# Anaesthesiaye/sound_event_detection_transformer

Measured on AMD Instinct MI355X. Metric: audio clips/sec training throughput (B=64, 10s@64-mel), higher is better.
Workload: dtype bf16; 1 GPU; URBAN-SED SEDT enc_layers=3 dec_at num_queries=10 B=64/GPU, 10 s @ 64-mel (B,1,500,64), full train step: fwd + Hungarian matching (device) + SetCriterion + bwd + clip 0.1 + AdamW, dropout 0.1; global_batch=64, parallelism=dp1

## Files before the change

### include/sedt_hip.h

```cpp
#ifndef SEDT_HIP_H
#define SEDT_HIP_H
#include <stddef.h>
#include <stdint.h>

#ifdef __cplusplus
extern "C" {
#endif

#define SEDT_F32 0
#define SEDT_BF16 1
#define SEDT_BF16X3 2
#define SEDT_I16 3

#define SEDT_ACT_NONE 0
#define SEDT_ACT_RELU 1
#define SEDT_ACT_SIGMOID 2

const char* sedt_last_error(void);
int sedt_version(void);

typedef struct SedtIgemm {
  int32_t M, N, K;
  const void* A;
  const void* B;
// ... 210 lines not shown
int sedt_bneck_fwd(const void* x, void* y, const void* w1_frag, const void* w2_frag, const void* w3_frag, const float* s1, const float* b1,
                   const float* s2, const float* b2, const float* s3, const float* b3, void* a_out, void* b_out, uint8_t* abits_out,
                   uint8_t* bbits_out, uint8_t* bits_out, int cin, int planes, int W, int B, int H, void* stream);
int sedt_bneck_bwd(const void* gy, void* gx, const void* w3t_frag, const void* w2t_frag, const void* w1t_frag, const uint8_t* abits,
                   const uint8_t* bbits, const uint8_t* xbits, void* gb_out, void* ga_out, int cin, int planes, int W, int B, int H,
                   void* stream);

int sedt_bneck3_ok(int cin, int planes, int W, int stride, int dil, int has_downsample, int B, int H, int dtype);
int sedt_bneck3_fwd(const void* x, void* y, const void* w1_frag, const void* w2_frag, const void* w3_frag, const float* s1, const float* b1,
                    const float* s2, const float* b2, const float* s3, const float* b3, void* a_out, void* b_out, uint8_t* abits_out,
                    uint8_t* bbits_out, uint8_t* bits_out, int B, int H, const SedtPrefetch* pf, void* stream);
int sedt_bneck3_bwd(const void* gy, void* gx, const void* w3t_frag, const void* w2t_frag, const void* w1t_frag, const uint8_t* abits,
                    const uint8_t* bbits, const uint8_t* xbits, void* gb_out, void* ga_out, int B, int H, const SedtPrefetch* pf,
                    void* stream);

int sedt_bneck0_ok(int cin, int planes, int W, int stride, int dil, int has_downsample, int dtype);
int sedt_bneck0_fwd(const void* x, void* y, const void* w1_frag, const void* w2_frag, const void* w3_frag, const void* wd_frag, const float* s1,
                    const float* b1, const float* s2, const float* b2, const float* s3, const float* b3, const float* sd, const float* bd,
                    void* a_out, void* b_out, uint8_t* abits_out, uint8_t* bbits_out, uint8_t* bits_out, int B, int H, void* stream);

int sedt_bneck2_ok(int cin, int planes, int W, int stride, int dil, int has_downsample, int dtype);
int sedt_bneck2_fwd(const void* x, void* y, const void* w1_frag, const void* w2_frag, const void* w3_frag, const void* wd_frag, const float* s1,
                    const float* b1, const float* s2, const float* b2, const float* s3, const float* b3, const float* sd, const float* bd,
                    void* a_out, void* b_out, uint8_t* bits_out, int B, int H, void* stream);

int sedt_heads_slab_ok(int D, int C1, int CA, int dtype);
int sedt_heads_fwd(const void* x, const float* wc, const float* bc, const void* w1_frag, const float* b1, const void* w2_frag,
                   const float* b2, const float* w3, const float* b3, const float* wa, const float* ba, float* cls, float* box, float* at,
                   void* h1, void* h2, int L, int B, int Qp, int C1, int CA, void* stream);
size_t sedt_heads_bwd_part_floats(int L, int B, int Qp, int C1, int CA);
int sedt_heads_bwd(const void* x, const void* h1, const void* h2, const float* box, const float* at, const float* g_cls,
                   const float* g_box, const float* g_at, const float* wc, const float* w3, const float* wa, const void* w2t_frag,
                   const void* w1t_frag, void* dhs, void* g_h1, void* g_h2, float* part, int L, int B, int Qp, int C1, int CA, void* stream);

int sedt_encoder_ffn_bwd(const void* gx2, const void* h, const void* x1, const float* mean2, const float* rstd2,
                         const float* gamma2, const void* w2t_frag, const void* w1t_frag, const void* wot_frag, void* g2, void* gh,
                         void* gx1, void* g1, void* gctx, float* ln_part, int B, int S, int FF, float drop_p, uint32_t seed_f,
                         uint32_t seed_o, const uint32_t* seed_ptr, void* stream);
int sedt_encoder_qkv_bwd(const void* dqk, const void* dv, const void* x, const float* mean1, const float* rstd1,
                         const float* gamma1, const void* gx1, const void* wint_frag, void* gx, float* ln_part, int B, int S,
                         void* stream);
int sedt_encoder_qkv_fwd(const void* x, const void* pos, const float* gamma, const float* beta, const void* w_in_frag,
                         const float* b_in, void* qk, void* v, void* xn, void* xnp, float* mean, float* rstd, int B, int S,
                         const SedtPrefetch* pf, void* stream);
int sedt_encoder_attn_ffn_fwd(const void* x, const void* qk, const void* v, const uint8_t* kpm, const void* w_o_frag,
                              const float* b_o, const float* gamma2, const float* beta2, const void* w1_frag, const float* b1,
                              const void* w2_frag, const float* b2, void* x2, void* ctx, float* lse, void* x1, float* mean2,
                              float* rstd2, void* x1n, void* h, int B, int S, int FF, float drop_p, uint32_t seed_attn,
                              uint32_t seed_o, uint32_t seed_h, uint32_t seed_f, const uint32_t* seed_ptr, void* stream);

int sedt_multi_gather(const SedtChunk* table, int nchunks, int mode, void* stream);
int sedt_multi_ema(const SedtChunk* table, int nchunks, float decay, const int32_t* guard , void* stream);
int sedt_multi_sumsq(const SedtChunk* table, int nchunks, float* partial, float* sumsq, int32_t* step_ptr ,
                     int32_t* guard , uint32_t* seed_word , void* stream);
int sedt_multi_adamw(const SedtChunk* table, int nchunks, const float* sumsq, float max_norm, float beta1, float beta2,
                     float eps, const int32_t* step_ptr , const int32_t* guard ,
                     void* stream);

#define SEDT_CRIT_MAXL 8
#define SEDT_CRIT_MAXOUT (4 * SEDT_CRIT_MAXL + 6)
#define SEDT_CRIT_MAXCARD 8192
typedef struct SedtCriterion {
  const float* logits;
  const float* boxes;
  const float* at;
  const float* tc;
// ... 189 lines not shown
```

### sound_event_detection_transformer_amd/_build.py

```python
import os
import shutil
import subprocess
from concurrent.futures import ThreadPoolExecutor

HERE = os.path.dirname(os.path.abspath(__file__))
CSRC = os.path.join(HERE, 'csrc')
LIB = os.path.join(HERE, 'libsedt_hip.so')
OBJ = os.path.join(HERE, '..', 'build', 'obj')
SOURCES = ['igemm.hip', 'igemm3.hip', 'wgrad3.hip', 'wgrad4.hip', 'misc.hip', 'stem.hip', 'conv3x3_c64.hip',
           'norm_attn.hip', 'attn_mfma.hip', 'attn_f32_mfma.hip', 'enc_slab.hip', 'heads_slab.hip', 'bneck.hip', 'bneck3.hip', 'criterion.hip', 'postproc.hip', 'input.hip', 'skinny.hip', 'split3.hip', 'pool_at.hip', 'metrics.hip', 'decode.hip', 'psds.hip', 'sweep.hip', 'stitch.hip', 'recmetrics.hip', 'recpsds.hip', 'mel.hip', 'resample.hip', 'clips.hip', 'mixplan.hip', 'host.cpp']
FLAGS = ['--offload-arch=gfx950', '-O3', '-std=c++17', '-fPIC', '-Wno-pass-failed']
if os.environ.get('SEDT_DEV_BUILD') == '1':
    FLAGS = FLAGS + ['-DSEDT_DEV']
    LIB = os.path.join(HERE, '..', 'build', 'dev', 'libsedt_hip_dev.so')
    OBJ = os.path.join(HERE, '..', 'build', 'dev', 'obj')


def source_stamp():
    import hashlib
    h = hashlib.sha256()
    files = [os.path.join(CSRC, f) for f in sorted(os.listdir(CSRC)) if f.endswith(('.hip', '.h', '.cpp'))]
    files.append(os.path.join(HERE, '..', 'include', 'sedt_hip.h'))
    for d, _, fs in sorted(os.walk(HERE)):
        if '__pycache__' in d or os.sep + 'csrc' in d:
            continue
        files += [os.path.join(d, f) for f in sorted(fs) if f.endswith('.py')]
    for f in files:
        h.update(os.path.relpath(f, HERE).encode())
        with open(f, 'rb') as fh:
            h.update(fh.read())
    return h.hexdigest()[:16]


def _headers():
    hs = [os.path.join(CSRC, f) for f in os.listdir(CSRC) if f.endswith('.h')]
    return hs + [os.path.join(HERE, '..', 'include', 'sedt_hip.h'), os.path.abspath(__file__)]


def _newer(target, deps):
    if not os.path.exists(target):
        return True
    t = os.path.getmtime(target)
    return any(os.path.getmtime(d) > t for d in deps if os.path.exists(d))
# ... 51 lines not shown
```

### sound_event_detection_transformer_amd/functional.py

```python
import torch
from torch.autograd import Function

from . import ops, packing, runtime
from .lib import F32, BF16
from .ops import ACT_NONE, ACT_RELU, ACT_SIGMOID, ConvGeom


def _dt_of(t):
    return F32 if t.dtype == torch.float32 else BF16


def _as(t, dt):
    want = torch.float32 if dt == F32 else torch.bfloat16
    t = t.contiguous()
    return t if t.dtype == want else ops.cast(t, dt)


def _wf(dt, w):
    return w if dt == F32 else ops.cast(w, BF16)


def _wb(dt, w):
    return ops.pack_conv(dt, w, want_fwd=False)[1]

# ... 415 lines not shown
    d_win = ops._sink(w_in, (3 * E, E))
    if d_win is None:
        d_win = torch.empty((3 * E, E), device=g_out.device, dtype=torch.float32)
    d_bin = torch.empty((3 * E,), device=g_out.device, dtype=torch.float32)
    wb = s['wb_in']
    g_q = g_k = g_v = None
    dgrads = []
    if s['same_qk']:
        ops.linear_wgrad(dt, dqk, s['q_in'], out=d_win[:2 * E], bias_out=d_bin[:2 * E], batch=batch)
        if need_q or need_k:
            dgrads.append(('q', dqk, wb[:, :2 * E]))
    else:
        ops.linear_wgrad(dt, dq, s['q_in'], out=d_win[:E], bias_out=d_bin[:E], batch=batch)
        ops.linear_wgrad(dt, dk, s['k_in'], out=d_win[E:2 * E], bias_out=d_bin[E:2 * E], batch=batch)
        if need_q:
            dgrads.append(('q', dq, wb[:, :E]))
        if need_k and not kv_fused:
            dgrads.append(('k', dk, wb[:, E:2 * E]))
    ops.linear_wgrad(dt, dv, s['v_in'], out=d_win[2 * E:], bias_out=d_bin[2 * E:], batch=batch)
    if kv_fused and not s['same_qk']:
        dgrads.append(('v', dkv, wb[:, E:], {} if res_kv is None else dict(res=res_kv, ldr=res_kv.stride(0))))
    elif need_v:
        dgrads.append(('v', dv, wb[:, 2 * E:]))
    if dgrads:
        got = dict(zip([d[0] for d in dgrads], ops.linear_group(dt, [(d[1], d[2], dict(d[3]) if len(d) > 3 else {}) for d in dgrads])))
        g_q, g_k, g_v = got.get('q'), got.get('k'), got.get('v')
    return g_q, g_k, g_v, d_win, d_bin, d_wo, d_bo


def _ffn_fwd(dt, x_in, w1, b1, w2, b2, res, p, seeds, train=True, out=None, act='relu'):
    sp = runtime.seed_ptr(x_in.device) if p > 0 else None
    wf1, wb1 = _prep_linear(dt, w1, train)
    wf2, wb2 = _prep_linear(dt, w2, train)
    if act == 'gelu':
        h_pre = ops.linear(dt, x_in, wf1, bias=b1)
        h = ops.gelu_fwd(dt, h_pre, p, seeds[0], sp)
        out = ops.linear(dt, h, wf2, out, bias=b2, drop_p=p, seed=seeds[1], seed_ptr=sp, res=res, ldr=res.stride(0))
        return out, dict(x_in=x_in, h=h, h_pre=h_pre, p=p, seeds=seeds, wb1=wb1, wb2=wb2)
    h = ops.linear(dt, x_in, wf1, bias=b1, act=ACT_RELU, drop_p=p, seed=seeds[0], seed_ptr=sp)
    out = ops.linear(dt, h, wf2, out, bias=b2, drop_p=p, seed=seeds[1], seed_ptr=sp, res=res, ldr=res.stride(0))
    return out, dict(x_in=x_in, h=h, p=p, seeds=seeds, wb1=wb1, wb2=wb2)


def _ffn_bwd(dt, s, g_out, w1, w2, res_for_gx=None, batch=None, g_dropped=None):
    p = s['p']
    if g_dropped is not None:
        g2 = g_dropped
    else:
        g2 = ops.dropout_grad(dt, g_out, p, s['seeds'][1], runtime.seed_ptr(g_out.device)) if p > 0 else g_out
    d_b2 = torch.empty((g2.shape[1],), device=g2.device, dtype=torch.float32)
    d_w2 = ops.linear_wgrad(dt, g2, s['h'], bias_out=d_b2, batch=batch, param=w2)
    if s.get('h_pre') is not None:
        gh = ops.gelu_bwd(dt, ops.linear(dt, g2, s['wb2']), s['h_pre'], p, s['seeds'][0], runtime.seed_ptr(g2.device) if p > 0 else None)
    else:
        gh = ops.linear(dt, g2, s['wb2'], mask=s['h'], ldm=s['h'].stride(0), alpha=1.0 / (1.0 - p) if p > 0 else 1.0)
    d_b1 = torch.empty((gh.shape[1],), device=gh.device, dtype=torch.float32)
    d_w1 = ops.linear_wgrad(dt, gh, s['x_in'], bias_out=d_b1, batch=batch, param=w1)
    if res_for_gx is not None:
        gx = ops.linear(dt, gh, s['wb1'], res=res_for_gx, ldr=res_for_gx.stride(0))
    else:
        gx = ops.linear(dt, gh, s['wb1'])
    return gx, d_w1, d_b1, d_w2, d_b2


class EncoderLayerFn(Function):

    @staticmethod
    def forward(ctx, x, pos, kpm, amask, cfg, *P):
        dt = cfg['dt']
        (w_in, b_in, w_o, b_o, w1, b1, w2, b2, g1, be1, g2, be2) = P
        B, S, H = cfg['B'], cfg['S'], cfg['H']
        p = cfg['dropout'] if cfg['training'] else 0.0
        seeds = [runtime.next_seed() for _ in range(4)]
        x = _as(x, dt)
        pos = _as(pos, dt)
        sv = {}
        tr = any(ctx.needs_input_grad)
        fr = None
# ... 411 lines not shown
```

### sound_event_detection_transformer_amd/lib.py

```python
import ctypes as C
import os

import torch

HERE = os.path.dirname(os.path.abspath(__file__))
LIB_PATH = os.path.join(HERE, 'libsedt_hip.so')
if os.environ.get('SEDT_LIB_AB') and os.environ.get('SEDT_DEV') == '1':
    LIB_PATH = os.environ['SEDT_LIB_AB']

F32, BF16 = 0, 1
BF16X3 = 2
I16 = 3
RESAMPLE_BLK = 1024
RESAMPLE_DESC_WORDS = 6
CLIPS_MAXB = 1024
GEMM_X3 = False


def gemm_dtype(dtype):
    return BF16X3 if (dtype == F32 and GEMM_X3) else dtype
ACT_NONE, ACT_RELU, ACT_SIGMOID = 0, 1, 2
TORCH_DTYPE = {F32: torch.float32, BF16: torch.bfloat16}


# ... 115 lines not shown
    'sedt_spsedt_dec_in': (_i, [_vp, _vp, _vp, _vp, _vp, _i, _i, _i, _i, _i, _i, _f, _u32, _vp, _i, _vp]),
    'sedt_spsedt_dec_in_bwd': (_i, [_vp, _vp, _vp, _vp, _i, _i, _i, _i, _i, _i, _i, _vp]),
    'sedt_gelu_fwd': (_i, [_vp, _vp, _i64, _f, _u32, _vp, _i, _vp]),
    'sedt_gelu_bwd': (_i, [_vp, _vp, _vp, _i64, _f, _u32, _vp, _i, _vp]),
    'sedt_sigmoid_grad': (_i, [_vp, _vp, _vp, _i64, _vp]),
    'sedt_layernorm_fwd': (_i, [_vp, _vp, _vp, _vp, _vp, _vp, _vp, _vp, _i, _i, _i, _vp]),
    'sedt_layernorm_bwd': (_i, [_vp, _vp, _vp, _vp, _vp, _vp, _vp, _vp, _vp, _vp, _vp, _sz, _i, _i, _i, _vp]),
    'sedt_layernorm_bwd_scratch': (_sz, [_i, _i]),
    'sedt_layernorm_bwd_drop': (_i, [_vp, _vp, _vp, _vp, _vp, _vp, _vp, _vp, _vp, _vp, _vp, _vp, _sz, _i, _i, _vp, _f, _u32, _vp, _i, _vp]),
    'sedt_layernorm_bwd_final': (_i, [_vp, _i, _i, _vp, _vp, _vp]),
    'sedt_attention_fwd': (_i, [_vp, _i64, _vp, _i64, _vp, _i64, _vp, _i64, _vp, _vp, _vp, _i, _i, _i, _i, _f, _u32,
                                _vp, _i, _vp]),
    'sedt_attention_bwd': (_i, [_vp, _i64, _vp, _i64, _vp, _i64, _vp, _i64, _vp, _i64, _vp, _vp, _vp, _vp, _i64, _vp,
                                _i64, _vp, _i64, _i, _i, _i, _i, _f, _u32, _vp, _i, _vp]),
    'sedt_attention_describe': (_i, [_vp, _i64] * 8 + [_i, _i, _i, _f, _i, _i, C.c_char_p, _i]),
    'sedt_pack_frag': (_i, [_vp, _i, _i, _vp]),
    'sedt_encoder_slab_ok': (_i, [_i, _i, _i, _i, _i]),
    'sedt_encoder_qkv_fwd': (_i, [_vp] * 12 + [_i, _i, C.POINTER(SedtPrefetch), _vp]),
    'sedt_encoder_attn_ffn_fwd': (_i, [_vp] * 20 + [_i, _i, _i, _f, _u32, _u32, _u32, _u32, _vp, _vp]),
    'sedt_bneck_ok': (_i, [_i] * 7),
    'sedt_bneck3_ok': (_i, [_i] * 9),
    'sedt_bneck3_fwd': (_i, [_vp] * 16 + [_i, _i, C.POINTER(SedtPrefetch), _vp]),
    'sedt_bneck3_bwd': (_i, [_vp] * 10 + [_i, _i, C.POINTER(SedtPrefetch), _vp]),
    'sedt_bneck0_ok': (_i, [_i] * 7),
    'sedt_bneck2_ok': (_i, [_i] * 7),
    'sedt_bneck2_fwd': (_i, [_vp] * 17 + [_i, _i, _vp]),
    'sedt_bneck0_fwd': (_i, [_vp] * 19 + [_i, _i, _vp]),
    'sedt_bneck_fwd': (_i, [_vp] * 16 + [_i] * 5 + [_vp]),
    'sedt_bneck_bwd': (_i, [_vp] * 10 + [_i] * 5 + [_vp]),
    'sedt_heads_slab_ok': (_i, [_i, _i, _i, _i]),
    'sedt_heads_fwd': (_i, [_vp] * 16 + [_i] * 5 + [_vp]),
    'sedt_heads_bwd_part_floats': (_sz, [_i] * 5),
    'sedt_heads_bwd': (_i, [_vp] * 17 + [_i] * 5 + [_vp]),
    'sedt_encoder_ffn_bwd': (_i, [_vp] * 15 + [_i, _i, _i, _f, _u32, _u32, _vp, _vp]),
    'sedt_encoder_qkv_bwd': (_i, [_vp] * 10 + [_i, _i, _vp]),
    'sedt_posenc': (_i, [_vp, _vp, _i, _i, _i, _i, _i, _vp]),
    'sedt_mask_resize': (_i, [_vp, _vp, _i, _i, _i, _i, _i, _vp]),
    'sedt_bn_fold': (_i, [_vp, _vp, _vp, _vp, _vp, _vp, _i, _vp]),
    'sedt_pack_conv': (_i, [_vp, _i, _i, _i, _vp, _vp, _vp, _i, _vp]),
    'sedt_stem_prep': (_i, [_vp, _vp, _vp, _vp, _i, _vp]),
    'sedt_stem_im2col': (_i, [_vp, _vp, _i, _i, _i, _i, _vp]),
    'sedt_stem_conv0_grad': (_i, [_vp, _vp, _vp, _vp, _vp]),
    'sedt_conv3x3_c64': (_i, [_vp, _vp, _i, _vp, _vp, _i, _vp, _vp, _i, _i, _i, _i, _vp]),
    'sedt_stem_pool_fwd': (_i, [_vp, _vp, _vp, _vp, _vp, _vp, _vp, _i, _i, _i, _vp]),
    'sedt_stem_pool_wgrad_slabs': (_i, [_i, _i]),
    'sedt_stem_pool_wgrad': (_i, [_vp, _vp, _vp, _vp, _vp, _i, _i, _i, _i, _vp]),
    'sedt_maxpool_fwd': (_i, [_vp, _vp, _vp, _i, _i, _i, _i, _i, _vp]),
    'sedt_maxpool_bwd': (_i, [_vp, _vp, _vp, _vp, _i, _i, _i, _i, _i, _vp]),
    'sedt_maxpool_bwd_y': (_i, [_vp, _vp, _vp, _vp, _vp, _i, _i, _i, _i, _i, _vp]),
    'sedt_avgpool': (_i, [_vp, _vp, _i, _i, _i, _i, _vp]),
    'sedt_sumsq': (_i, [_vp, _i64, _vp, _vp, _sz, _i, _vp]),
    'sedt_sumsq_scratch': (_sz, [_i64]),
    'sedt_multi_bn_fold': (_i, [_vp, _i, _vp]),
    'sedt_multi_pack': (_i, [_vp, _i, _i, _i, _vp]),
    'sedt_multi_gather': (_i, [_vp, _i, _i, _vp]),
    'sedt_multi_ema': (_i, [_vp, _i, _f, _vp, _vp]),
    'sedt_multi_sumsq': (_i, [_vp, _i, _vp, _vp, _vp, _vp, _vp, _vp]),
    'sedt_multi_adamw': (_i, [_vp, _i, _vp, _f, _f, _f, _f, _vp, _vp, _vp]),
    'sedt_set_criterion_scratch': (_sz, [_i, _i, _i]),
    'sedt_set_criterion': (_i, [C.POINTER(SedtCriterion), _vp, _vp]),
    'sedt_set_criterion_bwd': (_i, [C.POINTER(SedtCriterion), _vp, _vp, _vp, _vp, _vp, _vp, _vp]),
    'sedt_match_targets': (_i, [C.POINTER(SedtMatch), _vp]),
    'sedt_feature_loss': (_i, [_vp, _vp, _vp, _vp, _vp, C.POINTER(C.c_int32), _vp, _i, _i, _i, _i, _i, _i, _vp, _vp, _vp, _vp, _vp, _vp, _vp]),
    'sedt_scale_layers': (_i, [_vp, _vp, _vp, _vp, C.POINTER(C.c_int32), _i, _i64, _vp]),
    'sedt_sum_f32': (_i, [_vp, _i, _vp, _vp]),
    'sedt_pool_at': (_i, [C.POINTER(SedtPoolAt), _vp, _vp]),
# ... 80 lines not shown
```

### sound_event_detection_transformer_amd/ops.py

```python
import ctypes as C

import os
import numpy as np
import torch

from . import lib as L
from .lib import F32, BF16, ACT_NONE, ACT_RELU, ACT_SIGMOID, TORCH_DTYPE, p as _p


class ConvGeom(object):
    __slots__ = ('Hi', 'Wi', 'Ci', 'Ho', 'Wo', 'Co', 'KH', 'KW', 'sh', 'sw', 'ph', 'pw', 'dh', 'dw')

    def __init__(self, Hi, Wi, Ci, Co, k=1, stride=1, pad=0, dil=1):
        self.Hi, self.Wi, self.Ci, self.Co = Hi, Wi, Ci, Co
        self.KH = self.KW = k
        self.sh = self.sw = stride
        self.ph = self.pw = pad
        self.dh = self.dw = dil
        self.Ho = (Hi + 2 * pad - dil * (k - 1) - 1) // stride + 1
        self.Wo = (Wi + 2 * pad - dil * (k - 1) - 1) // stride + 1

    @property
    def taps(self):
        return self.KH * self.KW
# ... 1218 lines not shown

HEADS_SLAB_MAX_ROWS = 12288


def heads_slab_ok(dtype, D, C1, CA, rows=0):
    return bool(SLAB_HEADS and dtype == BF16 and rows <= HEADS_SLAB_MAX_ROWS and L.load().sedt_heads_slab_ok(D, C1, CA, dtype))


def heads_fwd(x, wc, bc, w1f, b1, w2f, b2, w3, b3, wa, ba, Lh, B, Qp, train=True):
    _dev_check(x, wc, w3)
    rows, D = x.shape
    assert x.is_contiguous() and rows == Lh * B * Qp and wc.is_contiguous() and w3.is_contiguous() and (wa is None or wa.is_contiguous())
    C1, CA = wc.shape[0], 0 if wa is None else wa.shape[0]
    f32 = dict(device=x.device, dtype=torch.float32)
    cls, box = torch.empty((rows, C1), **f32), torch.empty((rows, 2), **f32)
    at = torch.empty((B, CA), **f32) if CA else None
    hh = (torch.empty_like(x), torch.empty_like(x)) if train else None
    L.check(L.load().sedt_heads_fwd(_p(x), _p(wc), _p(bc), _p(w1f), _p(b1), _p(w2f), _p(b2), _p(w3), _p(b3), _p(wa), _p(ba), _p(cls), _p(box),
                                    _p(at), _p(hh[0]) if hh else None, _p(hh[1]) if hh else None, Lh, B, Qp, C1, CA, L.stream_ptr()), 'heads_fwd')
    return cls, box, at, hh


def heads_bwd(x, h1, h2, box, at, g_cls, g_box, g_at, wc, w3, wa, w2t, w1t, Lh, B, Qp):
    rows, D = x.shape
    C1, CA = wc.shape[0], 0 if wa is None else wa.shape[0]
    dhs, g_h1, g_h2 = torch.empty_like(x), torch.empty_like(x), torch.empty_like(x)
    nsl = (rows + 31) // 32
    part = torch.empty((nsl, (C1 + CA + 2) * 257), device=x.device, dtype=torch.float32)
    for g in (g_cls, g_box, g_at):
        assert g is None or (g.dtype == torch.float32 and g.is_contiguous())
    L.check(L.load().sedt_heads_bwd(_p(x), _p(h1), _p(h2), _p(box), _p(at), _p(g_cls), _p(g_box), _p(g_at), _p(wc), _p(w3), _p(wa), _p(w2t),
                                    _p(w1t), _p(dhs), _p(g_h1), _p(g_h2), _p(part), Lh, B, Qp, C1, CA, L.stream_ptr()), 'heads_bwd')
    return dhs, g_h1, g_h2, part


def encoder_ffn_bwd(gx2, h, x1, mean2, rstd2, gamma2, w2t_frag, w1t_frag, wot_frag, B, S, drop_p=0.0, seeds=(0, 0), seed_ptr=None):
    _dev_check(gx2, h, x1)
    M, D = gx2.shape
    FF = h.shape[1]
    assert gx2.is_contiguous() and h.is_contiguous() and x1.is_contiguous() and M == B * S
    nsl = B * ((S + 31) // 32)
    g2 = torch.empty_like(gx2) if drop_p > 0 else None
    g1 = torch.empty_like(gx2) if drop_p > 0 else None
    gh = torch.empty_like(h)
    gx1, gctx = torch.empty_like(gx2), torch.empty_like(gx2)
    part = torch.empty((nsl, 2 * D), device=gx2.device, dtype=torch.float32)
    L.check(L.load().sedt_encoder_ffn_bwd(_p(gx2), _p(h), _p(x1), _p(mean2), _p(rstd2), _p(gamma2), _p(w2t_frag), _p(w1t_frag),
                                          _p(wot_frag), _p(g2), _p(gh), _p(gx1), _p(g1), _p(gctx), _p(part), B, S, FF, drop_p,
                                          seeds[0] & 0xffffffff, seeds[1] & 0xffffffff, _p(seed_ptr), L.stream_ptr()), 'encoder_ffn_bwd')
    return (g2 if g2 is not None else gx2), gh, gx1, (g1 if g1 is not None else gx1), gctx, part


def encoder_qkv_bwd(dqk, dv, x, mean1, rstd1, gamma1, gx1, wint_frag, B, S):
    _dev_check(dqk, dv, x, gx1)
    M, D = x.shape
    assert dqk.is_contiguous() and dv.is_contiguous() and x.is_contiguous() and gx1.is_contiguous() and M == B * S
    gx = torch.empty_like(x)
    part = torch.empty((B * ((S + 31) // 32), 2 * D), device=x.device, dtype=torch.float32)
    L.check(L.load().sedt_encoder_qkv_bwd(_p(dqk), _p(dv), _p(x), _p(mean1), _p(rstd1), _p(gamma1), _p(gx1), _p(wint_frag), _p(gx),
                                          _p(part), B, S, L.stream_ptr()), 'encoder_qkv_bwd')
    return gx, part


def posenc(dtype, mask_u8, D):
    B, H, W = mask_u8.shape
    pos = torch.empty((B, H * W, D), device=mask_u8.device, dtype=TORCH_DTYPE[dtype])
# ... 557 lines not shown
```

### sound_event_detection_transformer_amd/sedt/sedt.py

```python
import torch
from torch import nn

from .. import functional as Fn
from .. import ops, packing, runtime
from ..ops import ACT_NONE, ACT_RELU, ACT_SIGMOID
from ..utilities.utils import NestedTensor, nested_tensor_from_tensor_list


class HipLinear(nn.Linear):

    def forward(self, x, act=ACT_NONE, out_f32=False):
        lead = x.shape[:-1]
        y = Fn.LinearFn.apply(x.reshape(-1, x.shape[-1]), self.weight, self.bias, act, out_f32, runtime.compute_dtype())
        return y.view(*lead, self.out_features)


class HipConv1x1(nn.Conv2d):

    relu_input = False
    input_bits = None

    def forward(self, x):
        B, C, H, W = x.shape
        tok = x.permute(0, 2, 3, 1).reshape(B * H * W, C)
# ... 46 lines not shown
        self.dec_at = dec_at
        self.pooling = pooling
        if self.dec_at:
            self.query_embed = nn.Embedding(num_queries + 1, hidden_dim)
            self.weak_class_embed = HipLinear(hidden_dim, num_classes)
        else:
            self.query_embed = nn.Embedding(num_queries, hidden_dim)
        if self.pool_mode == 'attn':
            self.attn_dense_softmax = HipLinear(hidden_dim, num_classes)

    def pack_plan(self):
        dt, dev = runtime.compute_dtype(), self.query_embed.weight.device
        key = (dt, str(dev))
        plans = self.__dict__.setdefault('_plans', {})
        if key not in plans:
            def factory():
                body = self.backbone[0].body
                convs = []
                l34 = set(id(p_) for layer in (body.layer3, body.layer4) for p_ in layer.parameters())
                bn_only = [(body.conv1.weight, body.bn1.tensors())]
                for layer in (body.layer1, body.layer2, body.layer3, body.layer4):
                    for b in layer:
                        convs += [(b.conv1.weight, b.bn1.tensors()), (b.conv2.weight, b.bn2.tensors()), (b.conv3.weight, b.bn3.tensors())]
                        if b.downsample is not None:
                            convs.append((b.downsample[0].weight, b.downsample[1].tensors()))
                lin = [self.input_proj.weight]
                frags = []
                for l in self.transformer.encoder.layers:
                    lin += [l.self_attn.in_proj_weight, l.self_attn.out_proj.weight, l.linear1.weight, l.linear2.weight]
                    frags += [l.self_attn.in_proj_weight, l.self_attn.out_proj.weight, l.linear1.weight, l.linear2.weight]
                for l in self.transformer.decoder.layers:
                    lin += [l.self_attn.in_proj_weight, l.self_attn.out_proj.weight, l.multihead_attn.in_proj_weight,
                            l.multihead_attn.out_proj.weight, l.linear1.weight, l.linear2.weight]
                    frags += [l.self_attn.in_proj_weight, l.self_attn.out_proj.weight, l.multihead_attn.in_proj_weight,
                              l.multihead_attn.out_proj.weight, l.linear1.weight, l.linear2.weight]
                lin += [self.class_embed.weight] + [m.weight for m in self.bbox_embed.layers]
                frags += [m.weight for m in self.bbox_embed.layers[:2]]
                for name in ('weak_class_embed', 'patch2query', 'attn_dense_softmax'):
                    if hasattr(self, name):
                        lin.append(getattr(self, name).weight)
                if hasattr(self, 'feature_align'):
                    lin += [m.weight for m in self.feature_align.layers]
                cfr = [w for layer in (body.layer1, body.layer2, body.layer3) for b in layer if b.downsample is None
                       for w in (b.conv1.weight, b.conv2.weight, b.conv3.weight)]
                for b0 in (body.layer1[0], body.layer2[0]):
                    cfr += [b0.conv1.weight, b0.conv2.weight, b0.conv3.weight, b0.downsample[0].weight]
                if ops.IGEMM_BREG:
                    have = set(id(w) for w in cfr)
                    cfr += [w for w, _ in convs if id(w) not in have and id(w) in l34]
                return packing.PackPlan(dt, dev, convs, lin, bn_only, frags, cfr)
            plans[key] = packing.PlanSet(factory)
        return plans[key]

    def forward(self, samples):
        with self.pack_plan():
            return self._forward(samples)

    def _forward(self, samples):
        if isinstance(samples, (list, torch.Tensor)):
            samples = nested_tensor_from_tensor_list(samples)
        features, pos = self.backbone(samples)
        src, mask = features[-1].decompose()
        assert mask is not None
        out = {}
        hs, memory = self.transformer(self.input_proj(src), mask, self.query_embed.weight, pos[-1], enc_at_embed=None)
        q0 = 1 if self.dec_at else 0
        b = self.bbox_embed.layers
        wa = (self.weak_class_embed.weight, self.weak_class_embed.bias) if self.dec_at else (None, None)
# ... 553 lines not shown
```

Before: 13070 clips/s.

## Fuse small-M transformer FFN pair into one split-FF kernel for fwd and bwd

Adds a fused kernel that computes linear1+ReLU+dropout and linear2+dropout+residual in one launch for small row counts (decoder FFN with few queries). Work is split across four FF-quarter blocks per 32-row slab, with the last-arriving block reducing the fp32 partials. A matching backward kernel fuses the dgrad through both linears and the ReLU mask, and weight grads still use the existing wgrad path. This targets launch overhead and the h round trip for tiny decoder GEMMs. It adds counter-based cross-block reduction and partial-buffer traffic, and drops fragment packing for the decoder attention weights.

```diff
diff --git a/include/sedt_hip.h b/include/sedt_hip.h
--- a/include/sedt_hip.h
+++ b/include/sedt_hip.h
@@ -266,6 +266,15 @@
 int sedt_heads_bwd(const void* x, const void* h1, const void* h2, const float* box, const float* at, const float* g_cls,
                    const float* g_box, const float* g_at, const float* wc, const float* w3, const float* wa, const void* w2t_frag,
                    const void* w1t_frag, void* dhs, void* g_h1, void* g_h2, float* part, int L, int B, int Qp, int C1, int CA, void* stream);
+
+int sedt_ffn_pair_ok(int D, int FF, int dtype);
+size_t sedt_ffn_pair_part_floats(int M);
+int sedt_ffn_pair_fwd(const void* x, int64_t ldx, const void* res, int64_t ldr, const void* w1_frag, const float* b1, const void* w2_frag,
+                      const float* b2, void* h, void* out, int64_t ldo, float* part, uint32_t* cnt, int M, int FF, float drop_p,
+                      uint32_t seed_h, uint32_t seed_f, const uint32_t* seed_ptr, void* stream);
+int sedt_ffn_pair_bwd(const void* g, int64_t ldg, int g_is_dropped, const void* h, const void* w2t_frag, const void* w1t_frag, void* g2,
+                      void* gh, const void* res, int64_t ldr, void* gx, float* part, uint32_t* cnt, int M, int FF, float drop_p,
+                      uint32_t seed_f, const uint32_t* seed_ptr, void* stream);
 
 int sedt_encoder_ffn_bwd(const void* gx2, const void* h, const void* x1, const float* mean2, const float* rstd2,
                          const float* gamma2, const void* w2t_frag, const void* w1t_frag, const void* wot_frag, void* g2, void* gh,
diff --git a/sound_event_detection_transformer_amd/_build.py b/sound_event_detection_transformer_amd/_build.py
--- a/sound_event_detection_transformer_amd/_build.py
+++ b/sound_event_detection_transformer_amd/_build.py
@@ -8,7 +8,7 @@
 LIB = os.path.join(HERE, 'libsedt_hip.so')
 OBJ = os.path.join(HERE, '..', 'build', 'obj')
 SOURCES = ['igemm.hip', 'igemm3.hip', 'wgrad3.hip', 'wgrad4.hip', 'misc.hip', 'stem.hip', 'conv3x3_c64.hip',
-           'norm_attn.hip', 'attn_mfma.hip', 'attn_f32_mfma.hip', 'enc_slab.hip', 'heads_slab.hip', 'bneck.hip', 'bneck3.hip', 'criterion.hip', 'postproc.hip', 'input.hip', 'skinny.hip', 'split3.hip', 'pool_at.hip', 'metrics.hip', 'decode.hip', 'psds.hip', 'sweep.hip', 'stitch.hip', 'recmetrics.hip', 'recpsds.hip', 'mel.hip', 'resample.hip', 'clips.hip', 'mixplan.hip', 'host.cpp']
+           'norm_attn.hip', 'attn_mfma.hip', 'attn_f32_mfma.hip', 'enc_slab.hip', 'ffn_pair.hip', 'heads_slab.hip', 'bneck.hip', 'bneck3.hip', 'criterion.hip', 'postproc.hip', 'input.hip', 'skinny.hip', 'split3.hip', 'pool_at.hip', 'metrics.hip', 'decode.hip', 'psds.hip', 'sweep.hip', 'stitch.hip', 'recmetrics.hip', 'recpsds.hip', 'mel.hip', 'resample.hip', 'clips.hip', 'mixplan.hip', 'host.cpp']
 FLAGS = ['--offload-arch=gfx950', '-O3', '-std=c++17', '-fPIC', '-Wno-pass-failed']
 if os.environ.get('SEDT_DEV_BUILD') == '1':
     FLAGS = FLAGS + ['-DSEDT_DEV']
diff --git a/sound_event_detection_transformer_amd/csrc/ffn_pair.hip b/sound_event_detection_transformer_amd/csrc/ffn_pair.hip
--- /dev/null
+++ b/sound_event_detection_transformer_amd/csrc/ffn_pair.hip
@@ -0,0 +1,357 @@
+#include "slab.h"
+
+namespace sedt {
+
+using slab::u32x4;
+using slab::XP;
+
+constexpr int FP_D = 256;
+constexpr int FP_NQ = 4;
+constexpr int FP_NT = 512;
+constexpr int FP_SP = FP_D + 4;
+constexpr size_t FP_TILES = (size_t)2 * 32 * XP * sizeof(bf16_t);
+constexpr size_t FP_SUMT = (size_t)32 * FP_SP * sizeof(float);
+constexpr size_t FP_FLAG_OFF = FP_TILES > FP_SUMT ? FP_TILES : FP_SUMT;
+constexpr size_t FP_LDS = FP_FLAG_OFF + 16;
+
+struct FfnPairArgs {
+  const bf16_t* xin; long ldx;
+  const bf16_t* res; long ldr;
+  const u32x4* wa;
+  const u32x4* wb;
+  const float* b1; const float* b2;
+  bf16_t* h;
+  bf16_t* out; long ldo;
+  bf16_t* g2;
+  bf16_t* gh;
+  float* part;
+  unsigned* cnt;
+  int M, FF;
+  int drop_in;
+  float drop_p;
+  uint32_t thresh, seed_h, seed_f;
+  const uint32_t* seed_ptr;
+};
+
+__device__ __forceinline__ int quarter_tile(int FF, int g, int i) { return ((g >> 1) * (FF >> 7) + i) * 2 + (g & 1); }
+
+__device__ __forceinline__ void load_w_first(u32x4 (&w)[16], const u32x4* __restrict__ W, int tile, int lane) {
+  const u32x4* p = W + (long)tile * (16 * 64) + lane;
+#pragma unroll
+  for (int u = 0; u < 16; ++u) w[u] = p[u * 64];
+}
+
+__device__ __forceinline__ void load_w_second(u32x4 (&w)[16], const u32x4* __restrict__ W, int FF, int g, int i0, int nv, int wave, int lane) {
+  const u32x4* p = W + (long)wave * (FF / 16) * 64 + lane;
+#pragma unroll
+  for (int ii = 0; ii < 8; ++ii) {
+    if (ii < nv) {
+      const long ks = (long)quarter_tile(FF, g, i0 + ii) * 2;
+      w[2 * ii] = p[ks * 64];
+      w[2 * ii + 1] = p[(ks + 1) * 64];
+    }
+  }
+}
+
+__device__ __forceinline__ void gemm_first(f32x16& acc, const u32x4 (&w)[16], const bf16_t* xs, int lane) {
+  const bf16_t* xrow = xs + (lane & 31) * XP + 8 * (lane >> 5);
+#pragma unroll
+  for (int u = 0; u < 16; ++u)
+    acc = __builtin_amdgcn_mfma_f32_32x32x16_bf16(__builtin_bit_cast(bf16x8, w[u]), *reinterpret_cast<const bf16x8*>(xrow + u * 16), acc, 0, 0, 0);
+}
+
+__device__ __forceinline__ void gemm_second(f32x16& acc, const u32x4 (&w)[16], const bf16_t* hs, int nv, int lane) {
+  const bf16_t* hrow = hs + (lane & 31) * XP + 8 * (lane >> 5);
+#pragma unroll
+  for (int ii = 0; ii < 8; ++ii) {
+    if (ii < nv) {
+#pragma unroll
+      for (int q = 0; q < 2; ++q)
+        acc = __builtin_amdgcn_mfma_f32_32x32x16_bf16(__builtin_bit_cast(bf16x8, w[2 * ii + q]),
+                                                      *reinterpret_cast<const bf16x8*>(hrow + ii * 32 + q * 16), acc, 0, 0, 0);
+    }
+  }
+}
+
+__device__ __forceinline__ long part_off(int nslab, int g, int sl, int tile, int g4, int lane) {
+  return (((((long)g * nslab + sl) * 8 + tile) * 4 + g4) * 64 + lane) * 4;
+}
+
+__device__ __forceinline__ void store_partial(const f32x16& acc, float* __restrict__ part, int nslab, int g, int sl, int wave, int lane) {
+#pragma unroll
+  for (int g4 = 0; g4 < 4; ++g4)
+    slab::store_sc1(part + part_off(nslab, g, sl, wave, g4, lane),
+                    slab::f32x4_t{acc[4 * g4 + 0], acc[4 * g4 + 1], acc[4 * g4 + 2], acc[4 * g4 + 3]});
+}
+
+__device__ __forceinline__ void sum_partials(const float* __restrict__ part, int nslab, int sl, float* SUM, int wave, int lane) {
+  const int n = lane & 31, hf = lane >> 5;
+  float4 v[4];
+#pragma unroll
+  for (int g4 = 0; g4 < 4; ++g4) v[g4] = *reinterpret_cast<const float4*>(part + part_off(nslab, 0, sl, wave, g4, lane));
+#pragma unroll
+  for (int g = 1; g < FP_NQ; ++g) {
+#pragma unroll
+    for (int g4 = 0; g4 < 4; ++g4) {
+      const float4 a = *reinterpret_cast<const float4*>(part + part_off(nslab, g, sl, wave, g4, lane));
+      v[g4].x += a.x; v[g4].y += a.y; v[g4].z += a.z; v[g4].w += a.w;
+    }
+  }
+#pragma unroll
+  for (int g4 = 0; g4 < 4; ++g4) *reinterpret_cast<float4*>(SUM + n * FP_SP + wave * 32 + 8 * g4 + 4 * hf) = v[g4];
+}
+
+template <bool TRAIN>
+__global__ __launch_bounds__(FP_NT) void ffn_pair_fwd_kernel(const FfnPairArgs a) {
+  extern __shared__ __attribute__((aligned(16))) unsigned char smem[];
+  bf16_t* X = reinterpret_cast<bf16_t*>(smem);
+  bf16_t* H = X + 32 * XP;
+  float* SUM = reinterpret_cast<float*>(smem);
+  unsigned* FLAG = reinterpret_cast<unsigned*>(smem + FP_FLAG_OFF);
+  const int tid = threadIdx.x, lane = tid & 63, wave = tid >> 6, n = lane & 31, hf = lane >> 5;
+  const int nslab = (a.M + 31) / 32;
+  const int g = blockIdx.x & 3, sl = blockIdx.x >> 2;
+  const int T = a.FF >> 7;
+  const long row0 = (long)sl * 32;
+  const int nvalid = min(32, a.M - (int)row0);
+  const float inv_keep = a.thresh ? 1.f / (1.f - a.drop_p) : 1.f;
+  const uint32_t sd_off = a.seed_ptr ? *a.seed_ptr : 0u;
+  const uint32_t sd_h = a.seed_h + sd_off, sd_f = a.seed_f + sd_off;
+  uint4 xr[2];
+#pragma unroll
+  for (int q = 0; q < 2; ++q) {
+    const int u = tid + q * FP_NT, r = u >> 5, c = (u & 31) * 8;
+    xr[q] = r < nvalid ? *reinterpret_cast<const uint4*>(a.xin + (row0 + r) * a.ldx + c) : make_uint4(0, 0, 0, 0);
+  }
+  u32x4 w1[16], w2[16];
+  if (wave < T) load_w_first(w1, a.wa, quarter_tile(a.FF, g, wave), lane);
+  load_w_second(w2, a.wb, a.FF, g, 0, min(8, T), wave, lane);
+  slab::issue_fence();
+#pragma unroll
+  for (int q = 0; q < 2; ++q) {
+    const int u = tid + q * FP_NT, r = u >> 5, c = (u & 31) * 8;
+    *reinterpret_cast<uint4*>(X + r * XP + c) = xr[q];
+  }
+  __syncthreads();
+  f32x16 acc2;
+#pragma unroll
+  for (int r = 0; r < 16; ++r) acc2[r] = 0.f;
+  for (int i0 = 0; i0 < T; i0 += 8) {
+    const int nv = min(8, T - i0);
+    if (wave < nv) {
+      const int t1 = quarter_tile(a.FF, g, i0 + wave);
+      float4 bb[4];
+      slab::load_feat4(bb, a.b1, t1, hf);
+      f32x16 acc;
+#pragma unroll
+      for (int r = 0; r < 16; ++r) acc[r] = 0.f;
+      gemm_first(acc, w1, X, lane);
+      if (i0 + 8 + wave < T) load_w_first(w1, a.wa, quarter_tile(a.FF, g, i0 + 8 + wave), lane);
+#pragma unroll
+      for (int g4 = 0; g4 < 4; ++g4) {
+        const int fl = 8 * g4 + 4 * hf;
+        const float bv[4] = {bb[g4].x, bb[g4].y, bb[g4].z, bb[g4].w};
+        const uint64_t idx = (uint64_t)(row0 + n) * a.FF + t1 * 32 + fl;
+        uint32_t keep = 0xfu;
+        if (a.thresh) keep = drop_keep4(slab::inner0(sd_h), 0u, sd_h, idx, a.thresh);
+        VecT<bf16_t, 4> o;
+#pragma unroll
+        for (int e = 0; e < 4; ++e) {
+          float v = fmaxf(acc[4 * g4 + e] + bv[e], 0.f);
+          if (a.thresh) v = (keep >> e & 1u) ? v * inv_keep : 0.f;
+          o.v[e] = (bf16_t)(n < nvalid ? v : 0.f);
+        }
+        *reinterpret_cast<VecT<bf16_t, 4>*>(H + n * XP + wave * 32 + fl) = o;
+      }
+    }
+    __syncthreads();
+    if (TRAIN) {
+      for (int u = tid; u < nv * 32 * 4; u += FP_NT) {
+        const int ii = u >> 7, r = (u >> 2) & 31, c = (u & 3) * 8;
+        if (r < nvalid)
+          *reinterpret_cast<uint4*>(a.h + (row0 + r) * a.FF + quarter_tile(a.FF, g, i0 + ii) * 32 + c) =
+              *reinterpret_cast<const uint4*>(H + r * XP + ii * 32 + c);
+      }
+    }
+    gemm_second(acc2, w2, H, nv, lane);
+    if (i0 + 8 < T) load_w_second(w2, a.wb, a.FF, g, i0 + 8, min(8, T - i0 - 8), wave, lane);
+    __syncthreads();
+  }
+  store_partial(acc2, a.part, nslab, g, sl, wave, lane);
+  if (!slab::arrive_last(a.cnt + sl, FP_NQ, FLAG, tid)) return;
+  sum_partials(a.part, nslab, sl, SUM, wave, lane);
+  __syncthreads();
+  for (int u = tid; u < 1024; u += FP_NT) {
+    const int r = u >> 5, c = (u & 31) * 8;
+    if (r >= nvalid) continue;
+    const float4 s0 = *reinterpret_cast<const float4*>(SUM + r * FP_SP + c), s1 = *reinterpret_cast<const float4*>(SUM + r * FP_SP + c + 4);
+    const float4 b0 = *reinterpret_cast<const float4*>(a.b2 + c), b1v = *reinterpret_cast<const float4*>(a.b2 + c + 4);
+    float v[8] = {s0.x + b0.x, s0.y + b0.y, s0.z + b0.z, s0.w + b0.w, s1.x + b1v.x, s1.y + b1v.y, s1.z + b1v.z, s1.w + b1v.w};
+    const bf16x8 xv = *reinterpret_cast<const bf16x8*>(a.res + (row0 + r) * a.ldr + c);
+    if (a.thresh) {
+      const uint32_t keep = drop_keep8(sd_f, (uint64_t)(row0 + r) * FP_D + c, a.thresh);
+#pragma unroll
+      for (int e = 0; e < 8; ++e) v[e] = (keep >> e & 1u) ? v[e] * inv_keep : 0.f;
+    }
+    bf16x8 o;
+#pragma unroll
+    for (int e = 0; e < 8; ++e) o[e] = (bf16_t)(v[e] + (float)xv[e]);
+    *reinterpret_cast<bf16x8*>(a.out + (row0 + r) * a.ldo + c) = o;
+  }
+}
+
+__global__ __launch_bounds__(FP_NT) void ffn_pair_bwd_kernel(const FfnPairArgs a) {
+  extern __shared__ __attribute__((aligned(16))) unsigned char smem[];
+  bf16_t* G2 = reinterpret_cast<bf16_t*>(smem);
+  bf16_t* GH = G2 + 32 * XP;
+  float* SUM = reinterpret_cast<float*>(smem);
+  unsigned* FLAG = reinterpret_cast<unsigned*>(smem + FP_FLAG_OFF);
+  const int tid = threadIdx.x, lane = tid & 63, wave = tid >> 6, n = lane & 31, hf = lane >> 5;
+  const int nslab = (a.M + 31) / 32;
+  const int g = blockIdx.x & 3, sl = blockIdx.x >> 2;
+  const int T = a.FF >> 7;
+  const long row0 = (long)sl * 32;
+  const int nvalid = min(32, a.M - (int)row0);
+  const float inv_keep = a.thresh ? 1.f / (1.f - a.drop_p) : 1.f;
+  const uint32_t sd_f = a.seed_f + (a.seed_ptr ? *a.seed_ptr : 0u);
+  bf16x8 gin[2];
+#pragma unroll
+  for (int q = 0; q < 2; ++q) {
+    const int u = tid + q * FP_NT, r = u >> 5, c = (u & 31) * 8;
+#pragma unroll
+    for (int e = 0; e < 8; ++e) gin[q][e] = (bf16_t)0.f;
+    if (r < nvalid) gin[q] = *reinterpret_cast<const bf16x8*>(a.xin + (row0 + r) * a.ldx + c);
+  }
+  u32x4 w2t[16], w1t[16];
+  if (wave < T) load_w_first(w2t, a.wa, quarter_tile(a.FF, g, wave), lane);
+  load_w_second(w1t, a.wb, a.FF, g, 0, min(8, T), wave, lane);
+  slab::issue_fence();
+#pragma unroll
+  for (int q = 0; q < 2; ++q) {
+    const int u = tid + q * FP_NT, r = u >> 5, c = (u & 31) * 8;
+    bf16x8 o = gin[q];
+    if (a.drop_in && r < nvalid) {
+      const long base = (row0 + r) * FP_D + c;
+      const uint32_t keep = drop_keep8(sd_f, (uint64_t)base, a.thresh);
+#pragma unroll
+      for (int e = 0; e < 8; ++e) o[e] = (keep >> e & 1u) ? (bf16_t)((float)gin[q][e] * inv_keep) : (bf16_t)0.f;
+      if (a.g2 && g == 0) *reinterpret_cast<bf16x8*>(a.g2 + base) = o;
+    }
+    *reinterpret_cast<bf16x8*>(G2 + r * XP + c) = o;
+  }
+  __syncthreads();
+  f32x16 acc2;
+#pragma unroll
+  for (int r = 0; r < 16; ++r) acc2[r] = 0.f;
+  for (int i0 = 0; i0 < T; i0 += 8) {
+    const int nv = min(8, T - i0);
+    if (wave < nv) {
+      const int t2 = quarter_tile(a.FF, g, i0 + wave);
+      VecT<bf16_t, 4> hv[4];
+#pragma unroll
+      for (int g4 = 0; g4 < 4; ++g4) {
+        hv[g4] = VecT<bf16_t, 4>{};
+        if (n < nvalid) hv[g4] = *reinterpret_cast<const VecT<bf16_t, 4>*>(a.h + (row0 + n) * a.FF + t2 * 32 + 8 * g4 + 4 * hf);
+      }
+      f32x16 acc;
+#pragma unroll
+      for (int r = 0; r < 16; ++r) acc[r] = 0.f;
+      gemm_first(acc, w2t, G2, lane);
+      if (i0 + 8 + wave < T) load_w_first(w2t, a.wa, quarter_tile(a.FF, g, i0 + 8 + wave), lane);
+#pragma unroll
+      for (int g4 = 0; g4 < 4; ++g4) {
+        VecT<bf16_t, 4> o;
+#pragma unroll
+        for (int e = 0; e < 4; ++e) o.v[e] = (bf16_t)(((float)hv[g4].v[e] > 0.f ? acc[4 * g4 + e] : 0.f) * inv_keep);
+        *reinterpret_cast<VecT<bf16_t, 4>*>(GH + n * XP + wave * 32 + 8 * g4 + 4 * hf) = o;
+      }
+    }
+    __syncthreads();
+    for (int u = tid; u < nv * 32 * 4; u += FP_NT) {
+      const int ii = u >> 7, r = (u >> 2) & 31, c = (u & 3) * 8;
+      if (r < nvalid)
+        *reinterpret_cast<uint4*>(a.gh + (row0 + r) * a.FF + quarter_tile(a.FF, g, i0 + ii) * 32 + c) =
+            *reinterpret_cast<const uint4*>(GH + r * XP + ii * 32 + c);
+    }
+    gemm_second(acc2, w1t, GH, nv, lane);
+    if (i0 + 8 < T) load_w_second(w1t, a.wb, a.FF, g, i0 + 8, min(8, T - i0 - 8), wave, lane);
+    __syncthreads();
+  }
+  store_partial(acc2, a.part, nslab, g, sl, wave, lane);
+  if (!slab::arrive_last(a.cnt + sl, FP_NQ, FLAG, tid)) return;
+  sum_partials(a.part, nslab, sl, SUM, wave, lane);
+  __syncthreads();
+  for (int u = tid; u < 1024; u += FP_NT) {
+    const int r = u >> 5, c = (u & 31) * 8;
+    if (r >= nvalid) continue;
+    const float4 s0 = *reinterpret_cast<const float4*>(SUM + r * FP_SP + c), s1 = *reinterpret_cast<const float4*>(SUM + r * FP_SP + c + 4);
+    float v[8] = {s0.x, s0.y, s0.z, s0.w, s1.x, s1.y, s1.z, s1.w};
+    if (a.res) {
+      const bf16x8 xv = *reinterpret_cast<const bf16x8*>(a.res + (row0 + r) * a.ldr + c);
+#pragma unroll
+      for (int e = 0; e < 8; ++e) v[e] += (float)xv[e];
+    }
+    bf16x8 o;
+#pragma unroll
+    for (int e = 0; e < 8; ++e) o[e] = (bf16_t)v[e];
+    *reinterpret_cast<bf16x8*>(a.out + (row0 + r) * a.ldo + c) = o;
+  }
+}
+
+static int ffn_pair_launch(bool bwd, bool train, const FfnPairArgs& a, hipStream_t st) {
+  static_assert(FP_LDS <= 64 * 1024, "LDS");
+  const int grid = ((a.M + 31) / 32) * FP_NQ;
+  if (bwd) hipLaunchKernelGGL(ffn_pair_bwd_kernel, dim3(grid), dim3(FP_NT), FP_LDS, st, a);
+  else if (train) hipLaunchKernelGGL(ffn_pair_fwd_kernel<true>, dim3(grid), dim3(FP_NT), FP_LDS, st, a);
+  else hipLaunchKernelGGL(ffn_pair_fwd_kernel<false>, dim3(grid), dim3(FP_NT), FP_LDS, st, a);
+  return check_launch(bwd ? "ffn_pair_bwd" : "ffn_pair_fwd");
+}
+
+static bool aligned16(const void* p) { return (reinterpret_cast<uintptr_t>(p) & 15u) == 0; }
+
+}
+
+using namespace sedt;
+
+extern "C" int sedt_ffn_pair_ok(int D, int FF, int dtype) { return dtype == SEDT_BF16 && D == FP_D && FF >= 256 && FF % 256 == 0; }
+
+extern "C" size_t sedt_ffn_pair_part_floats(int M) { return (size_t)FP_NQ * ((size_t)(M + 31) / 32) * 32 * FP_D; }
+
+extern "C" int sedt_ffn_pair_fwd(const void* x, int64_t ldx, const void* res, int64_t ldr, const void* w1_frag, const float* b1,
+                                 const void* w2_frag, const float* b2, void* h, void* out, int64_t ldo, float* part, uint32_t* cnt, int M,
+                                 int FF, float drop_p, uint32_t seed_h, uint32_t seed_f, const uint32_t* seed_ptr, void* stream) {
+  SEDT_REQUIRE(x && res && w1_frag && b1 && w2_frag && b2 && out && part && cnt, "ffn_pair_fwd: null pointer");
+  SEDT_REQUIRE(M >= 1 && sedt_ffn_pair_ok(FP_D, FF, SEDT_BF16), "ffn_pair_fwd: FF = %d outside the envelope", FF);
+  SEDT_REQUIRE(drop_p >= 0.f && drop_p < 1.f, "ffn_pair_fwd: drop_p out of range");
+  SEDT_REQUIRE(ldx >= FP_D && ldr >= FP_D && ldo >= FP_D && ldx % 8 == 0 && ldr % 8 == 0 && ldo % 8 == 0, "ffn_pair_fwd: row strides");
+  SEDT_REQUIRE(aligned16(x) && aligned16(res) && aligned16(out) && aligned16(h) && aligned16(part) && aligned16(b1) && aligned16(b2) &&
+                   aligned16(w1_frag) && aligned16(w2_frag),
+               "ffn_pair_fwd: operands must be 16-byte aligned");
+  FfnPairArgs a{};
+  a.xin = (const bf16_t*)x; a.ldx = ldx; a.res = (const bf16_t*)res; a.ldr = ldr; a.wa = (const u32x4*)w1_frag; a.wb = (const u32x4*)w2_frag;
+  a.b1 = b1; a.b2 = b2; a.h = (bf16_t*)h; a.out = (bf16_t*)out; a.ldo = ldo; a.part = part; a.cnt = cnt; a.M = M; a.FF = FF;
+  a.drop_p = drop_p; a.thresh = drop_p > 0.f ? drop_threshold(drop_p) : 0u;
+  a.seed_h = seed_h; a.seed_f = seed_f; a.seed_ptr = seed_ptr;
+  return ffn_pair_launch(false, h != nullptr, a, reinterpret_cast<hipStream_t>(stream));
+}
+
+extern "C" int sedt_ffn_pair_bwd(const void* g, int64_t ldg, int g_is_dropped, const void* h, const void* w2t_frag, const void* w1t_frag,
+                                 void* g2, void* gh, const void* res, int64_t ldr, void* gx, float* part, uint32_t* cnt, int M, int FF,
+                                 float drop_p, uint32_t seed_f, const uint32_t* seed_ptr, void* stream) {
+  SEDT_REQUIRE(g && h && w2t_frag && w1t_frag && gh && gx && part && cnt, "ffn_pair_bwd: null pointer");
+  SEDT_REQUIRE(M >= 1 && sedt_ffn_pair_ok(FP_D, FF, SEDT_BF16), "ffn_pair_bwd: FF = %d outside the envelope", FF);
+  SEDT_REQUIRE(drop_p >= 0.f && drop_p < 1.f, "ffn_pair_bwd: drop_p out of range");
+  const bool drop_in = drop_p > 0.f && !g_is_dropped;
+  SEDT_REQUIRE(!drop_in || g2, "ffn_pair_bwd: the dropped gradient g2 has to be written (the weight gradient reads it)");
+  SEDT_REQUIRE(ldg >= FP_D && ldg % 8 == 0 && (!res || (ldr >= FP_D && ldr % 8 == 0)), "ffn_pair_bwd: row strides");
+  SEDT_REQUIRE(aligned16(g) && aligned16(h) && aligned16(g2) && aligned16(gh) && aligned16(res) && aligned16(gx) && aligned16(part) &&
+                   aligned16(w2t_frag) && aligned16(w1t_frag),
+               "ffn_pair_bwd: operands must be 16-byte aligned");
+  FfnPairArgs a{};
+  a.xin = (const bf16_t*)g; a.ldx = ldg; a.res = (const bf16_t*)res; a.ldr = ldr; a.wa = (const u32x4*)w2t_frag; a.wb = (const u32x4*)w1t_frag;
+  a.h = (bf16_t*)const_cast<void*>(h); a.out = (bf16_t*)gx; a.ldo = FP_D; a.g2 = drop_in ? (bf16_t*)g2 : nullptr; a.gh = (bf16_t*)gh;
+  a.part = part; a.cnt = cnt; a.M = M; a.FF = FF; a.drop_in = drop_in ? 1 : 0; a.drop_p = drop_p;
+  a.thresh = drop_p > 0.f ? drop_threshold(drop_p) : 0u;
+  a.seed_f = seed_f; a.seed_ptr = seed_ptr;
+  return ffn_pair_launch(true, true, a, reinterpret_cast<hipStream_t>(stream));
+}
diff --git a/sound_event_detection_transformer_amd/functional.py b/sound_event_detection_transformer_amd/functional.py
--- a/sound_event_detection_transformer_amd/functional.py
+++ b/sound_event_detection_transformer_amd/functional.py
@@ -471,6 +471,14 @@
     sp = runtime.seed_ptr(x_in.device) if p > 0 else None
     wf1, wb1 = _prep_linear(dt, w1, train)
     wf2, wb2 = _prep_linear(dt, w2, train)
+    pair = None
+    if ops.ffn_pair_ok(dt, x_in.shape[1], w1.shape[0], x_in.shape[0], act):
+        fr = [packing.lookup_frag(w) for w in (w1, w2)]
+        if all(f is not None for f in fr):
+            pair = dict(w1=fr[0][0], w2=fr[1][0], w1t=fr[0][1], w2t=fr[1][1])
+    if pair is not None and ops.FFN_PAIR_FWD:
+        out, h = ops.ffn_pair_fwd(x_in, pair['w1'], b1, pair['w2'], b2, res, p, seeds, sp, out=out, train=train)
+        return out, dict(x_in=x_in, h=h, p=p, seeds=seeds, wb1=wb1, wb2=wb2, pair=pair)
     if act == 'gelu':
         h_pre = ops.linear(dt, x_in, wf1, bias=b1)
         h = ops.gelu_fwd(dt, h_pre, p, seeds[0], sp)
@@ -478,11 +486,21 @@
         return out, dict(x_in=x_in, h=h, h_pre=h_pre, p=p, seeds=seeds, wb1=wb1, wb2=wb2)
     h = ops.linear(dt, x_in, wf1, bias=b1, act=ACT_RELU, drop_p=p, seed=seeds[0], seed_ptr=sp)
     out = ops.linear(dt, h, wf2, out, bias=b2, drop_p=p, seed=seeds[1], seed_ptr=sp, res=res, ldr=res.stride(0))
-    return out, dict(x_in=x_in, h=h, p=p, seeds=seeds, wb1=wb1, wb2=wb2)
+    return out, dict(x_in=x_in, h=h, p=p, seeds=seeds, wb1=wb1, wb2=wb2, pair=pair)
 
 
 def _ffn_bwd(dt, s, g_out, w1, w2, res_for_gx=None, batch=None, g_dropped=None):
     p = s['p']
+    if s.get('pair') is not None and ops.FFN_PAIR and ops.FFN_PAIR_BWD:
+        g = g_dropped if g_dropped is not None else g_out
+        gx, gh, g2 = ops.ffn_pair_bwd(g, s['h'], s['pair']['w2t'], s['pair']['w1t'], p, s['seeds'][1],
+                                      runtime.seed_ptr(g.device) if p > 0 else None, g_is_dropped=g_dropped is not None,
+                                      res_for_gx=res_for_gx)
+        d_b2 = torch.empty((g2.shape[1],), device=g2.device, dtype=torch.float32)
+        d_w2 = ops.linear_wgrad(dt, g2, s['h'], bias_out=d_b2, batch=batch, param=w2)
+        d_b1 = torch.empty((gh.shape[1],), device=gh.device, dtype=torch.float32)
+        d_w1 = ops.linear_wgrad(dt, gh, s['x_in'], bias_out=d_b1, batch=batch, param=w1)
+        return gx, d_w1, d_b1, d_w2, d_b2
     if g_dropped is not None:
         g2 = g_dropped
     else:
diff --git a/sound_event_detection_transformer_amd/lib.py b/sound_event_detection_transformer_amd/lib.py
--- a/sound_event_detection_transformer_amd/lib.py
+++ b/sound_event_detection_transformer_amd/lib.py
@@ -171,6 +171,10 @@
     'sedt_heads_fwd': (_i, [_vp] * 16 + [_i] * 5 + [_vp]),
     'sedt_heads_bwd_part_floats': (_sz, [_i] * 5),
     'sedt_heads_bwd': (_i, [_vp] * 17 + [_i] * 5 + [_vp]),
+    'sedt_ffn_pair_ok': (_i, [_i, _i, _i]),
+    'sedt_ffn_pair_part_floats': (_sz, [_i]),
+    'sedt_ffn_pair_fwd': (_i, [_vp, _i64, _vp, _i64, _vp, _vp, _vp, _vp, _vp, _vp, _i64, _vp, _vp, _i, _i, _f, _u32, _u32, _vp, _vp]),
+    'sedt_ffn_pair_bwd': (_i, [_vp, _i64, _i, _vp, _vp, _vp, _vp, _vp, _vp, _i64, _vp, _vp, _vp, _i, _i, _f, _u32, _vp, _vp]),
     'sedt_encoder_ffn_bwd': (_i, [_vp] * 15 + [_i, _i, _i, _f, _u32, _u32, _vp, _vp]),
     'sedt_encoder_qkv_bwd': (_i, [_vp] * 10 + [_i, _i, _vp]),
     'sedt_posenc': (_i, [_vp, _vp, _i, _i, _i, _i, _i, _vp]),
diff --git a/sound_event_detection_transformer_amd/ops.py b/sound_event_detection_transformer_amd/ops.py
--- a/sound_event_detection_transformer_amd/ops.py
+++ b/sound_event_detection_transformer_amd/ops.py
@@ -1274,6 +1274,68 @@
     L.check(L.load().sedt_heads_bwd(_p(x), _p(h1), _p(h2), _p(box), _p(at), _p(g_cls), _p(g_box), _p(g_at), _p(wc), _p(w3), _p(wa), _p(w2t),
                                     _p(w1t), _p(dhs), _p(g_h1), _p(g_h2), _p(part), Lh, B, Qp, C1, CA, L.stream_ptr()), 'heads_bwd')
     return dhs, g_h1, g_h2, part
+
+
+FFN_PAIR = _dev_env('SEDT_FFN_PAIR', '1') != '0'
+FFN_PAIR_FWD = _dev_env('SEDT_FFN_PAIR_FWD', '1') != '0'
+FFN_PAIR_BWD = _dev_env('SEDT_FFN_PAIR_BWD', '1') != '0'
+FFN_PAIR_MAX_ROWS = int(_dev_env('SEDT_FFN_PAIR_MAX_ROWS', '1024'))
+_FFN_PAIR_SLABS = 1024
+_ffn_pair_cnt = {}
+
+
+def ffn_pair_ok(dtype, D, FF, M, act='relu'):
+    return bool(FFN_PAIR and dtype == BF16 and act == 'relu' and M <= FFN_PAIR_MAX_ROWS
+                and L.load().sedt_ffn_pair_ok(D, FF, dtype))
+
+
+def _ffn_pair_ws(ref, M):
+    assert (M + 31) // 32 <= _FFN_PAIR_SLABS, 'ffn_pair: more than %d rows' % (32 * _FFN_PAIR_SLABS)
+    key = (ref.device.index, torch.cuda.current_stream(ref.device).cuda_stream)
+    cnt = _ffn_pair_cnt.get(key)
+    if cnt is None:
+        cnt = _ffn_pair_cnt[key] = torch.zeros((_FFN_PAIR_SLABS,), device=ref.device, dtype=torch.int32)
+    part = torch.empty((L.load().sedt_ffn_pair_part_floats(M),), device=ref.device, dtype=torch.float32)
+    return part, cnt
+
+
+def ffn_pair_fwd(x, w1_frag, b1, w2_frag, b2, res, drop_p=0.0, seeds=(0, 0), seed_ptr=None, out=None, h=None, train=True):
+    _dev_check(x, res, w1_frag, w2_frag)
+    M, D = x.shape
+    FF = b1.shape[0]
+    assert x.stride(1) == 1 and res.stride(1) == 1 and res.shape == x.shape and x.dtype == torch.bfloat16 and res.dtype == torch.bfloat16
+    if out is None:
+        out = torch.empty((M, D), device=x.device, dtype=torch.bfloat16)
+    assert out.shape == x.shape and out.stride(1) == 1 and out.dtype == torch.bfloat16
+    if train and h is None:
+        h = torch.empty((M, FF), device=x.device, dtype=torch.bfloat16)
+    assert h is None or (h.is_contiguous() and h.shape == (M, FF) and h.dtype == torch.bfloat16)
+    part, cnt = _ffn_pair_ws(x, M)
+    L.check(L.load().sedt_ffn_pair_fwd(_p(x), x.stride(0), _p(res), res.stride(0), _p(w1_frag), _p(b1), _p(w2_frag), _p(b2),
+                                       _p(h) if train else None, _p(out), out.stride(0), _p(part), _p(cnt), M, FF, drop_p,
+                                       seeds[0] & 0xffffffff, seeds[1] & 0xffffffff, _p(seed_ptr), L.stream_ptr()), 'ffn_pair_fwd')
+    return out, (h if train else None)
+
+
+def ffn_pair_bwd(g, h, w2t_frag, w1t_frag, drop_p=0.0, seed=0, seed_ptr=None, g_is_dropped=False, res_for_gx=None, g2=None, gh=None, gx=None):
+    _dev_check(g, h, w2t_frag, w1t_frag)
+    M, D = g.shape
+    FF = h.shape[1]
+    assert g.stride(1) == 1 and g.dtype == torch.bfloat16 and h.is_contiguous() and h.dtype == torch.bfloat16 and h.shape[0] == M
+    assert res_for_gx is None or (res_for_gx.stride(1) == 1 and res_for_gx.shape == g.shape and res_for_gx.dtype == torch.bfloat16)
+    drop_in = drop_p > 0 and not g_is_dropped
+    if drop_in and g2 is None:
+        g2 = torch.empty((M, D), device=g.device, dtype=torch.bfloat16)
+    if gh is None:
+        gh = torch.empty((M, FF), device=g.device, dtype=torch.bfloat16)
+    if gx is None:
+        gx = torch.empty((M, D), device=g.device, dtype=torch.bfloat16)
+    assert gh.is_contiguous() and gh.shape == (M, FF) and gx.is_contiguous() and gx.shape == (M, D) and (not drop_in or (g2.is_contiguous() and g2.shape == (M, D)))
+    part, cnt = _ffn_pair_ws(g, M)
+    L.check(L.load().sedt_ffn_pair_bwd(_p(g), g.stride(0), int(bool(g_is_dropped)), _p(h), _p(w2t_frag), _p(w1t_frag), _p(g2) if drop_in else None,
+                                       _p(gh), _p(res_for_gx), res_for_gx.stride(0) if res_for_gx is not None else 0, _p(gx), _p(part), _p(cnt),
+                                       M, FF, drop_p, seed & 0xffffffff, _p(seed_ptr), L.stream_ptr()), 'ffn_pair_bwd')
+    return gx, gh, (g2 if drop_in else g)
 
 
 def encoder_ffn_bwd(gx2, h, x1, mean2, rstd2, gamma2, w2t_frag, w1t_frag, wot_frag, B, S, drop_p=0.0, seeds=(0, 0), seed_ptr=None):
diff --git a/sound_event_detection_transformer_amd/sedt/sedt.py b/sound_event_detection_transformer_amd/sedt/sedt.py
--- a/sound_event_detection_transformer_amd/sedt/sedt.py
+++ b/sound_event_detection_transformer_amd/sedt/sedt.py
@@ -102,8 +102,7 @@
                 for l in self.transformer.decoder.layers:
                     lin += [l.self_attn.in_proj_weight, l.self_attn.out_proj.weight, l.multihead_attn.in_proj_weight,
                             l.multihead_attn.out_proj.weight, l.linear1.weight, l.linear2.weight]
-                    frags += [l.self_attn.in_proj_weight, l.self_attn.out_proj.weight, l.multihead_attn.in_proj_weight,
-                              l.multihead_attn.out_proj.weight, l.linear1.weight, l.linear2.weight]
+                    frags += [l.linear1.weight, l.linear2.weight]
                 lin += [self.class_embed.weight] + [m.weight for m in self.bbox_embed.layers]
                 frags += [m.weight for m in self.bbox_embed.layers[:2]]
                 for name in ('weak_class_embed', 'patch2query', 'attn_dense_softmax'):
```

Measured after the change: 13140 clips/s (median of 6 runs). No clear change (+0.6%).
